# ryienh/gnn-ops-benchmark

Measured on AMD Instinct MI355X. Metric: scatter_add effective HBM GB/s (algorithmic bytes / wall time, cold: index partition + bucketed segment reduce per call), higher is better.
Workload: dtype f32; 1 GPU; c2 (BASELINE configs[1]): torch_scatter.scatter_add(src[E,D], index[E], dim=0, dim_size=N), N=10000000 E=50000000 D=128 fp32, layout R

## Files before the change

gnn-ops-benchmark_amd/csrc/bucket.hip:

```cpp
#include "common.h"
#include "hub.h"
#include "sort_engine.h"

namespace {

constexpr int BSHIFT = 8, BROWS = 1 << BSHIFT;
constexpr int THREADS = 256, WAVES = THREADS / 64;
constexpr int ROUNDS = 16, CAP = THREADS * ROUNDS;
constexpr int U = 8;
constexpr bool NT = true;

inline size_t align_up(size_t v, size_t a) { return (v + a - 1) / a * a; }
inline int key_bits(int64_t N) {
    int bits = 1;
    while (bits < 32 && ((int64_t)1 << bits) < N) ++bits;
    return bits;
}

__global__ void bucket_bounds_kernel(const uint32_t* __restrict__ keys, int64_t E, int64_t NB, int32_t* __restrict__ bptr) {
    const int64_t b = (int64_t)blockIdx.x * blockDim.x + threadIdx.x;
    if (b > NB) return;
    int64_t lo = 0, hi = E;
    while (lo < hi) {
        const int64_t mid = (lo + hi) >> 1;
// ... 337 lines not shown
    if (hub_ws && E > hub::T_HUB) {
        const hub::Layout hl = hub::layout(E, K, want_arg);
        if (hub_ws_bytes >= hl.total) {
            hw = hub::make_ws(hub_ws, hl, E, want_arg);
            if (gnnops_memset_async(hw.counters, 0, 8, stream) != hipSuccess) return gnnops_check_launch("hub memset");
            hub_on = 1;
        }
    }
    hipLaunchKernelGGL((bucket_reduce_kernel<T, R>), dim3(grid), dim3(THREADS), 0, stream, (const T*)src, keys, vals, bptr,
                       (T*)out, arg_out, E, K, N, NB, gshift, kchunks, init_from_out, is_mean, hw, hub_on, spare_keys,
                       spare_vals);
    if (hub_on)
        hub::launch_pass<T, R, true>((const T*)src, nullptr, keys, vals, (T*)out, arg_out, hw, E, K, gshift, kchunks,
                                     init_from_out, is_mean, stream);
    return gnnops_check_launch("scatter_rows_oneshot");
}

template <typename T>
int dispatch_bucket(int reduce, const void* src, const uint32_t* keys, const uint32_t* vals, const int32_t* bptr, void* out,
                    int64_t* arg_out, int64_t E, int64_t K, int64_t N, int64_t NB, int init_from_out, hipStream_t stream,
                    void* hw = nullptr, size_t hb = 0, uint32_t* sk = nullptr, uint32_t* sv = nullptr) {
    switch (reduce) {
        case GNNOPS_SUM: return launch_bucket<T, GNNOPS_SUM>(src, keys, vals, bptr, out, nullptr, E, K, N, NB, init_from_out, 0, stream, hw, hb, sk, sv);
        case GNNOPS_MEAN: return launch_bucket<T, GNNOPS_SUM>(src, keys, vals, bptr, out, nullptr, E, K, N, NB, init_from_out, 1, stream, hw, hb, sk, sv);
        case GNNOPS_MUL: return launch_bucket<T, GNNOPS_MUL>(src, keys, vals, bptr, out, nullptr, E, K, N, NB, init_from_out, 0, stream, hw, hb, sk, sv);
        case GNNOPS_MIN: return launch_bucket<T, GNNOPS_MIN>(src, keys, vals, bptr, out, arg_out, E, K, N, NB, init_from_out, 0, stream, hw, hb, sk, sv);
        case GNNOPS_MAX: return launch_bucket<T, GNNOPS_MAX>(src, keys, vals, bptr, out, arg_out, E, K, N, NB, init_from_out, 0, stream, hw, hb, sk, sv);
    }
    gnnops_set_error("scatter_rows_oneshot: unknown reduce %d", reduce);
    return GNNOPS_EINVAL;
}

struct Layout {
    size_t keys_a, keys_b, vals_a, vals_b, tile_hist, digit_total, bptr, total;
};
inline Layout layout(int64_t E, int64_t N) {
    Layout l{};
    const size_t tiles = (size_t)gnnops_cdiv(E > 0 ? E : 1, sortengine::TILE);
    size_t o = 0;
    l.keys_a = o; o += align_up((size_t)E * 4, 256);
    l.keys_b = o; o += align_up((size_t)E * 4, 256);
    l.vals_a = o; o += align_up((size_t)E * 4, 256);
    l.vals_b = o; o += align_up((size_t)E * 4, 256);
    l.tile_hist = o; o += align_up(256 * tiles * 4, 256);
    l.digit_total = o; o += 256 * 4;
    l.bptr = o; o += align_up(((size_t)gnnops_cdiv(N, BROWS) + 1) * 4, 256);
    l.total = o;
    return l;
}

inline int64_t sentinel_key(int64_t N) { return gnnops_cdiv(N, BROWS) * BROWS; }
inline int partition_passes(int64_t N) { return (key_bits(sentinel_key(N) + 1) - BSHIFT + 7) / 8; }

__global__ void window_keys_kernel(const int64_t* __restrict__ index, uint32_t* __restrict__ keys, int64_t E, int64_t lo,
                                   int64_t N, uint32_t sentinel) {
    for (int64_t e = (int64_t)blockIdx.x * blockDim.x + threadIdx.x; e < E; e += (int64_t)gridDim.x * blockDim.x) {
        const uint64_t d = (uint64_t)(index[e] - lo);
        keys[e] = d < (uint64_t)N ? (uint32_t)d : sentinel;
    }
}

inline bool oneshot_shape_ok(int64_t E, int64_t N) {
    return N > BROWS && E > 0 && E < ((int64_t)1 << 31) && N < ((int64_t)1 << 31);
}

}

extern "C" size_t gnnops_bucket_workspace_bytes(int64_t E, int64_t N) {
    if (E < 0 || N < 0) return 0;
    return layout(E, N).total;
}

namespace {
int partition_impl(const int64_t* index, int64_t E, int64_t lo, int64_t N, bool window, void* workspace,
                   size_t workspace_bytes, hipStream_t stream, const char* what) {
    GNNOPS_REQUIRE(E >= 0 && N >= 0, GNNOPS_EINVAL, "%s: negative size", what);
    GNNOPS_REQUIRE(oneshot_shape_ok(E, N), GNNOPS_EUNSUPPORTED, "%s: shape outside the bucketed form (E=%lld N=%lld)", what,
                   (long long)E, (long long)N);
    GNNOPS_REQUIRE(index, GNNOPS_EINVAL, "%s: null pointer", what);
    const Layout l = layout(E, N);
    GNNOPS_REQUIRE(workspace && workspace_bytes >= l.total, GNNOPS_EWORKSPACE, "%s: workspace %zu < %zu", what,
                   workspace_bytes, l.total);
    char* w = (char*)workspace;
    uint32_t* kbuf[2] = {(uint32_t*)(w + l.keys_a), (uint32_t*)(w + l.keys_b)};
    uint32_t* vbuf[2] = {(uint32_t*)(w + l.vals_a), (uint32_t*)(w + l.vals_b)};
    uint32_t* tile_hist = (uint32_t*)(w + l.tile_hist);
    uint32_t* digit_total = (uint32_t*)(w + l.digit_total);
    int32_t* bptr = (int32_t*)(w + l.bptr);
    const int tiles = (int)gnnops_cdiv(E, sortengine::TILE);
    const int passes = partition_passes(N);
    if (window) {
        const int grid = gnnops_grid_cap(gnnops_cdiv(E, 256), 256 * 16);
        hipLaunchKernelGGL(window_keys_kernel, dim3(grid), dim3(256), 0, stream, index, kbuf[1], E, lo, N,
                           (uint32_t)sentinel_key(N));
    }
    const uint32_t* kin = nullptr;
    const uint32_t* vin = nullptr;
    for (int p = 0; p < passes; ++p) {
        uint32_t* kout = kbuf[p & 1];
        uint32_t* vout = vbuf[p & 1];
        int rc;
        if (p == 0)
            rc = window ? sortengine::pass_first_u32(kbuf[1], kout, vout, E, BSHIFT, tile_hist, digit_total, tiles, stream)
                        : sortengine::pass_first_i64(index, kout, vout, E, BSHIFT, tile_hist, digit_total, tiles, stream);
        else
            rc = sortengine::pass_u32(kin, vin, kout, vout, E, BSHIFT + 8 * p, tile_hist, digit_total, tiles, stream);
        if (rc != GNNOPS_OK) return rc;
        kin = kout; vin = vout;
    }
    const int64_t NB = gnnops_cdiv(N, BROWS);
    hipLaunchKernelGGL(bucket_bounds_kernel, dim3((unsigned)gnnops_cdiv(NB + 1, 256)), dim3(256), 0, stream, kin, E, NB, bptr);
    return gnnops_check_launch(what);
}
}

extern "C" int gnnops_bucket_partition(const int64_t* index, int64_t E, int64_t N, void* workspace, size_t workspace_bytes,
                                       gnnops_stream_t s) {
    return partition_impl(index, E, 0, N, false, workspace, workspace_bytes, (hipStream_t)s, "bucket_partition");
}

extern "C" int gnnops_bucket_partition_window(const int64_t* index, int64_t E, int64_t lo, int64_t N, void* workspace,
                                              size_t workspace_bytes, gnnops_stream_t s) {
    return partition_impl(index, E, lo, N, true, workspace, workspace_bytes, (hipStream_t)s, "bucket_partition_window");
}

extern "C" int gnnops_bucket_layout(int64_t E, int64_t N, size_t* keys_offset, size_t* vals_offset, size_t* bptr_offset) {
    GNNOPS_REQUIRE(E >= 0 && N >= 0 && keys_offset && vals_offset && bptr_offset, GNNOPS_EINVAL, "bucket_layout: bad argument");
    const Layout l = layout(E, N);
    const int last = (partition_passes(N) - 1) & 1;
    *keys_offset = last ? l.keys_b : l.keys_a;
    *vals_offset = last ? l.vals_b : l.vals_a;
    *bptr_offset = l.bptr;
    return GNNOPS_OK;
}

extern "C" int gnnops_bucket_reduce(const void* src, const void* workspace, void* out, int64_t* arg_out, int64_t E, int64_t K,
                                    int64_t N, int dtype, int reduce, int init_from_out, gnnops_stream_t s) {
    return gnnops_bucket_reduce_hubs(src, workspace, out, arg_out, E, K, N, dtype, reduce, init_from_out, nullptr, 0, s);
}

extern "C" int gnnops_bucket_reduce_hubs(const void* src, const void* workspace, void* out, int64_t* arg_out, int64_t E,
                                         int64_t K, int64_t N, int dtype, int reduce, int init_from_out, void* hub_workspace,
                                         size_t hub_workspace_bytes, gnnops_stream_t s) {
    hipStream_t stream = (hipStream_t)s;
    GNNOPS_REQUIRE(E >= 0 && K >= 0 && N >= 0, GNNOPS_EINVAL, "bucket_reduce: negative size");
    GNNOPS_REQUIRE(!(reduce == GNNOPS_MEAN && init_from_out), GNNOPS_EINVAL, "bucket_reduce: mean cannot start from out");
    GNNOPS_REQUIRE(dtype == GNNOPS_F32 || dtype == GNNOPS_F16 || dtype == GNNOPS_BF16, GNNOPS_EINVAL,
                   "bucket_reduce: unknown dtype %d", dtype);
    const int vec = dtype == GNNOPS_F32 ? 4 : 8;
    const bool rows_ok = K > 0 && K % vec == 0 && (uintptr_t)src % 16 == 0 && (uintptr_t)out % 16 == 0 &&
                         (arg_out == nullptr || (uintptr_t)arg_out % 16 == 0);
    GNNOPS_REQUIRE(rows_ok && oneshot_shape_ok(E, N), GNNOPS_EUNSUPPORTED,
                   "bucket_reduce: shape outside the bucketed form (E=%lld K=%lld N=%lld)", (long long)E, (long long)K,
                   (long long)N);
    GNNOPS_REQUIRE(src && workspace && out, GNNOPS_EINVAL, "bucket_reduce: null pointer");
    const Layout l = layout(E, N);
// ... 42 lines not shown
    hub::Ws hw{};
    int hub_on = 0;
    if (hub_workspace && E > hub::T_HUB) {
        const hub::Layout hl = hub::layout(E, 0, false);
        if (hub_workspace_bytes >= hl.total) {
            hw = hub::make_ws(hub_workspace, hl, E, false);
            if (gnnops_memset_async(hw.counters, 0, 8, stream) != hipSuccess) return gnnops_check_launch("hub memset");
            hub_on = 1;
        }
    }
    uint32_t* sk = (uint32_t*)(const_cast<char*>(w) + (last ? l.keys_a : l.keys_b));
    uint32_t* sv = (uint32_t*)(const_cast<char*>(w) + (last ? l.vals_a : l.vals_b));
    hipLaunchKernelGGL((bucket_push_kernel<8>), dim3(grid), dim3(THREADS), 0, stream, (const char*)input, keys, vals, bptr,
                       (char*)out, N, NB, rowbytes, gshift, chunks, hw, hub_on, sk, sv);
    if (hub_on)
        hub::launch_push_pass(true, (const char*)input, nullptr, keys, vals, (char*)out, hw, rowbytes, gshift, chunks, stream);
    return gnnops_check_launch("bucket_select");
}

extern "C" int gnnops_scatter_rows_oneshot(const void* src, const int64_t* index, void* out, int64_t* arg_out, int64_t E,
                                           int64_t K, int64_t N, int dtype, int reduce, int init_from_out,
                                           void* workspace, size_t workspace_bytes, gnnops_stream_t s) {
    GNNOPS_REQUIRE(E >= 0 && K >= 0 && N >= 0, GNNOPS_EINVAL, "scatter_rows_oneshot: negative size");
    const int vec = dtype == GNNOPS_F32 ? 4 : 8;
    const bool rows_ok = K > 0 && K % vec == 0 && (uintptr_t)src % 16 == 0 && (uintptr_t)out % 16 == 0 &&
                         (arg_out == nullptr || (uintptr_t)arg_out % 16 == 0);
    GNNOPS_REQUIRE(rows_ok && oneshot_shape_ok(E, N), GNNOPS_EUNSUPPORTED,
                   "scatter_rows_oneshot: shape outside the one-shot form (E=%lld K=%lld N=%lld)", (long long)E,
                   (long long)K, (long long)N);
    const int rc = gnnops_bucket_partition(index, E, N, workspace, workspace_bytes, s);
    if (rc != GNNOPS_OK) return rc;
    return gnnops_bucket_reduce(src, workspace, out, arg_out, E, K, N, dtype, reduce, init_from_out, s);
}
```

gnn-ops-benchmark_amd/csrc/sort_engine.h:

```cpp
#pragma once
#include "common.h"

namespace sortengine {

constexpr int THREADS = 512;
constexpr int WAVES = THREADS / 64;
constexpr int ROUNDS = 16;
constexpr int TILE = WAVES * ROUNDS * 64;
constexpr int RADIX = 256;

template <typename T>
struct DstValSrc {
    const int64_t* idx;
    const T* val;
    int64_t n_dst;
    uint32_t sentinel;
};

int pass_first_i64(const int64_t* index, uint32_t* keys_out, uint32_t* vals_out, int64_t n, int shift,
                   uint32_t* tile_hist, uint32_t* digit_total, int num_tiles, hipStream_t stream);
int pass_u32(const uint32_t* keys_in, const uint32_t* vals_in, uint32_t* keys_out, uint32_t* vals_out, int64_t n,
             int shift, uint32_t* tile_hist, uint32_t* digit_total, int num_tiles, hipStream_t stream);
int pass_first_u32(const uint32_t* keys_in, uint32_t* keys_out, uint32_t* vals_out, int64_t n, int shift,
                   uint32_t* tile_hist, uint32_t* digit_total, int num_tiles, hipStream_t stream);
int pass_first_f32(const float* keys_in, uint32_t* keys_out, uint32_t* vals_out, int64_t n, int shift,
                   uint32_t* tile_hist, uint32_t* digit_total, int num_tiles, hipStream_t stream);
int pass_first_u64(const uint64_t* keys_in, uint64_t* keys_out, uint32_t* vals_out, int64_t n, int shift,
                   uint32_t* tile_hist, uint32_t* digit_total, int num_tiles, hipStream_t stream);
int pass_u64(const uint64_t* keys_in, const uint32_t* vals_in, uint64_t* keys_out, uint32_t* vals_out, int64_t n,
             int shift, uint32_t* tile_hist, uint32_t* digit_total, int num_tiles, hipStream_t stream);
int pass_first_dstval_f32(const DstValSrc<float>* desc, uint64_t* keys_out, uint32_t* vals_out, int64_t n, int shift,
                          uint32_t* tile_hist, uint32_t* digit_total, int num_tiles, hipStream_t stream);
int pass_first_dstval_f16(const DstValSrc<__half>* desc, uint64_t* keys_out, uint32_t* vals_out, int64_t n, int shift,
                          uint32_t* tile_hist, uint32_t* digit_total, int num_tiles, hipStream_t stream);
int pass_first_dstval_bf16(const DstValSrc<__hip_bfloat16>* desc, uint64_t* keys_out, uint32_t* vals_out, int64_t n, int shift,
                           uint32_t* tile_hist, uint32_t* digit_total, int num_tiles, hipStream_t stream);


}
```

gnn-ops-benchmark_amd/csrc/sort_engine.hip:

```cpp
#include "sort_engine_impl.h"

namespace sortengine {

int pass_first_i64(const int64_t* index, uint32_t* keys_out, uint32_t* vals_out, int64_t n, int shift,
                   uint32_t* tile_hist, uint32_t* digit_total, int num_tiles, hipStream_t stream) {
    return run_pass<KeyI64Low32, true, true>(index, nullptr, keys_out, vals_out, n, shift, tile_hist, digit_total,
                                             num_tiles, stream);
}

int pass_u32(const uint32_t* keys_in, const uint32_t* vals_in, uint32_t* keys_out, uint32_t* vals_out, int64_t n,
             int shift, uint32_t* tile_hist, uint32_t* digit_total, int num_tiles, hipStream_t stream) {
    return run_pass<KeyU32, false, true>(keys_in, vals_in, keys_out, vals_out, n, shift, tile_hist, digit_total,
                                         num_tiles, stream);
}

int pass_first_u32(const uint32_t* keys_in, uint32_t* keys_out, uint32_t* vals_out, int64_t n, int shift,
                   uint32_t* tile_hist, uint32_t* digit_total, int num_tiles, hipStream_t stream) {
    return run_pass<KeyU32, true, true>(keys_in, nullptr, keys_out, vals_out, n, shift, tile_hist, digit_total, num_tiles,
                                        stream);
}

int pass_first_f32(const float* keys_in, uint32_t* keys_out, uint32_t* vals_out, int64_t n, int shift,
                   uint32_t* tile_hist, uint32_t* digit_total, int num_tiles, hipStream_t stream) {
    return run_pass<KeyF32, true, true>(keys_in, nullptr, keys_out, vals_out, n, shift, tile_hist, digit_total,
                                        num_tiles, stream);
}

int pass_first_u64(const uint64_t* keys_in, uint64_t* keys_out, uint32_t* vals_out, int64_t n, int shift,
                   uint32_t* tile_hist, uint32_t* digit_total, int num_tiles, hipStream_t stream) {
    return run_pass<KeyU64, true, true>(keys_in, nullptr, keys_out, vals_out, n, shift, tile_hist, digit_total,
                                        num_tiles, stream);
}

int pass_u64(const uint64_t* keys_in, const uint32_t* vals_in, uint64_t* keys_out, uint32_t* vals_out, int64_t n,
             int shift, uint32_t* tile_hist, uint32_t* digit_total, int num_tiles, hipStream_t stream) {
    return run_pass<KeyU64, false, true>(keys_in, vals_in, keys_out, vals_out, n, shift, tile_hist, digit_total,
                                         num_tiles, stream);
}

int pass_first_dstval_f32(const DstValSrc<float>* desc, uint64_t* keys_out, uint32_t* vals_out, int64_t n, int shift,
                          uint32_t* tile_hist, uint32_t* digit_total, int num_tiles, hipStream_t stream) {
    return run_pass<KeyDstVal<float>, true, true>(desc, nullptr, keys_out, vals_out, n, shift, tile_hist, digit_total, num_tiles, stream);
}

int pass_first_dstval_f16(const DstValSrc<__half>* desc, uint64_t* keys_out, uint32_t* vals_out, int64_t n, int shift,
                          uint32_t* tile_hist, uint32_t* digit_total, int num_tiles, hipStream_t stream) {
    return run_pass<KeyDstVal<__half>, true, true>(desc, nullptr, keys_out, vals_out, n, shift, tile_hist, digit_total, num_tiles, stream);
}

int pass_first_dstval_bf16(const DstValSrc<__hip_bfloat16>* desc, uint64_t* keys_out, uint32_t* vals_out, int64_t n, int shift,
// ... 7 lines not shown
```

gnn-ops-benchmark_amd/csrc/sort_engine_impl.h:

```cpp
#pragma once
#include "common.h"
#include "sort_engine.h"

namespace sortengine {

constexpr int HIST_THREADS = 256;
constexpr int HIST_WAVES = HIST_THREADS / 64;

struct KeyI64Low32 {
    template <typename P> __device__ static inline P open(P p) { return p; }
    using In = int64_t;
    using Carry = uint32_t;
    __device__ static inline Carry load(const In* p, int64_t i) {
        int64_t v = p[i];
        asm("" : "+v"(v));
        return (uint32_t)v;
    }
    __device__ static inline uint32_t digit(Carry k, int shift) { return (k >> shift) & 255u; }
};
struct KeyU32 {
    template <typename P> __device__ static inline P open(P p) { return p; }
    using In = uint32_t;
    using Carry = uint32_t;
    __device__ static inline Carry load(const In* p, int64_t i) { return p[i]; }
// ... 23 lines not shown
        s.n_dst = (uint64_t)p->n_dst;
        s.sentinel = p->sentinel;
        return s;
    }
    __device__ static inline Carry load(const Src& s, int64_t i) {
        const uint64_t d = (uint64_t)s.idx[i];
        float v;
        if constexpr (sizeof(T) == 4) {
            v = *reinterpret_cast<const __attribute__((address_space(1))) float*>(s.val + i);
        } else {
            const uint16_t bits = *reinterpret_cast<const __attribute__((address_space(1))) uint16_t*>(s.val + i);
            T raw;
            __builtin_memcpy(&raw, &bits, 2);
            v = Elem<T>::load(&raw);
        }
        const uint32_t hi = d < s.n_dst ? (uint32_t)d : s.sentinel;
        return ((uint64_t)hi << 32) | (uint64_t)__float_as_uint(v);
    }
    __device__ static inline uint32_t digit(Carry k, int shift) { return (uint32_t)(k >> shift) & 255u; }
};
struct KeyF32 {
    template <typename P> __device__ static inline P open(P p) { return p; }
    using In = float;
    using Carry = uint32_t;
    __device__ static inline Carry load(const In* p, int64_t i) {
        uint32_t u = __float_as_uint(p[i]);
        if (u == 0x80000000u) u = 0u;
        if ((u & 0x7fffffffu) > 0x7f800000u) return 0xffffffffu;
        return (u & 0x80000000u) ? ~u : (u | 0x80000000u);
    }
    __device__ static inline uint32_t digit(Carry k, int shift) { return (k >> shift) & 255u; }
};

template <typename KA>
__global__ __launch_bounds__(HIST_THREADS) void hist_kernel(const typename KA::In* __restrict__ keys_arg, int64_t n,
                                                            int shift, uint32_t* __restrict__ tile_hist,
                                                            int num_tiles) {
    __shared__ uint32_t h[HIST_WAVES][RADIX];
    const int tid = threadIdx.x, wave = tid >> 6;
    for (int i = tid; i < HIST_WAVES * RADIX; i += HIST_THREADS) (&h[0][0])[i] = 0;
    __syncthreads();
    const int tile = (int)xcd_contiguous(blockIdx.x, gridDim.x);
    const int64_t base = (int64_t)tile * TILE;
    const int lim = (int)((n - base < TILE) ? (n - base) : TILE);
    constexpr int GROUPS = TILE / (HIST_THREADS * 4);
    const auto keys = KA::open(keys_arg);
    if (lim == TILE) {
        typename KA::Carry k[GROUPS][4];
#pragma unroll
        for (int g = 0; g < GROUPS; ++g)
#pragma unroll
            for (int j = 0; j < 4; ++j) k[g][j] = KA::load(keys, base + (int64_t)(g * HIST_THREADS + tid) * 4 + j);
#pragma unroll
        for (int g = 0; g < GROUPS; ++g)
#pragma unroll
            for (int j = 0; j < 4; ++j) atomicAdd(&h[wave][KA::digit(k[g][j], shift)], 1u);
    } else {
        for (int i = tid; i < lim; i += HIST_THREADS) atomicAdd(&h[wave][KA::digit(KA::load(keys, base + i), shift)], 1u);
    }
    __syncthreads();
    uint32_t t = 0;
#pragma unroll
    for (int w = 0; w < HIST_WAVES; ++w) t += h[w][tid];
    tile_hist[(size_t)tid * num_tiles + tile] = t;
}

__global__ __launch_bounds__(HIST_THREADS) void scan_kernel(uint32_t* __restrict__ tile_hist, int num_tiles,
                                                            uint32_t* __restrict__ digit_total) {
    __shared__ uint32_t s_tmp[HIST_WAVES];
    uint32_t* row = tile_hist + (size_t)blockIdx.x * num_tiles;
    uint32_t carry = 0;
    constexpr int IPT = 8;
    for (int base = 0; base < num_tiles; base += HIST_THREADS * IPT) {
        uint32_t v[IPT];
        uint32_t sum = 0;
        const int i0 = base + threadIdx.x * IPT;
#pragma unroll
        for (int j = 0; j < IPT; ++j) {
            v[j] = (i0 + j < num_tiles) ? row[i0 + j] : 0u;
            sum += v[j];
        }
        uint32_t tot;
        uint32_t off = carry + block_excl_scan_u32<HIST_WAVES>(sum, s_tmp, &tot);
#pragma unroll
        for (int j = 0; j < IPT; ++j) {
            if (i0 + j < num_tiles) row[i0 + j] = off;
            off += v[j];
        }
        carry += tot;
    }
    if (threadIdx.x == 0) digit_total[blockIdx.x] = carry;
}

template <typename KA, bool IMPLICIT_VALS, bool WRITE_KEYS>
__global__ __launch_bounds__(THREADS, (sizeof(typename KA::Carry) == 4 ? 4 : 2)) void scatter_kernel(const typename KA::In* __restrict__ keys_arg,
                                                          const uint32_t* __restrict__ vals_in,
                                                          typename KA::Carry* __restrict__ keys_out,
                                                          uint32_t* __restrict__ vals_out, int64_t n, int shift,
                                                          const uint32_t* __restrict__ tile_hist_scanned,
                                                          const uint32_t* __restrict__ digit_total, int num_tiles) {
    using Carry = typename KA::Carry;
    constexpr bool PACKED = sizeof(Carry) == 4;
    __shared__ __attribute__((aligned(16))) unsigned char s_image[TILE * (sizeof(Carry) + 4)];
    __shared__ uint32_t s_whist[WAVES][RADIX];
    __shared__ uint32_t s_glob[RADIX];
    __shared__ uint32_t s_tmp[WAVES];
    uint64_t* s_pairs = reinterpret_cast<uint64_t*>(s_image);
    Carry* s_keys = reinterpret_cast<Carry*>(s_image);
    uint32_t* s_vals = reinterpret_cast<uint32_t*>(s_image + TILE * sizeof(Carry));

    const int tid = threadIdx.x, wave = tid >> 6, lane = tid & 63;
    for (int i = tid; i < WAVES * RADIX; i += THREADS) (&s_whist[0][0])[i] = 0;
    __syncthreads();

    const int tile = (int)xcd_contiguous(blockIdx.x, gridDim.x);
    const int64_t base = (int64_t)tile * TILE;
    const int64_t wave_base = base + (int64_t)wave * ROUNDS * 64;
    const uint64_t lanes_below = (lane == 0) ? 0ull : (~0ull >> (64 - lane));
    uint32_t* whist = &s_whist[wave][0];

    Carry key[ROUNDS];
    uint32_t val[ROUNDS];
    const auto keys_in = KA::open(keys_arg);
    if (base + TILE <= n) {
#pragma unroll
        for (int r = 0; r < ROUNDS; ++r) {
            const int64_t i = wave_base + r * 64 + lane;
            key[r] = KA::load(keys_in, i);
            if (!IMPLICIT_VALS) val[r] = vals_in[i];
        }
    } else {
#pragma unroll
        for (int r = 0; r < ROUNDS; ++r) {
            const int64_t i = wave_base + r * 64 + lane;
// ... 61 lines not shown
        if (i < n) {
            const uint32_t d = KA::digit(key[r], shift);
            const uint32_t pos = whist[d] + rank[r];
            const uint32_t v = IMPLICIT_VALS ? (uint32_t)i : val[r];
            if constexpr (PACKED) {
                s_pairs[pos] = ((uint64_t)v << 32) | (uint64_t)(uint32_t)key[r];
            } else {
                s_keys[pos] = key[r];
                s_vals[pos] = v;
            }
        }
    }
    __syncthreads();

    const int lim = (int)((n - base < TILE) ? (n - base) : TILE);
#pragma unroll 4
    for (int i = tid; i < lim; i += THREADS) {
        Carry k;
        uint32_t v;
        if constexpr (PACKED) {
            const uint64_t p = s_pairs[i];
            k = (Carry)(uint32_t)p;
            v = (uint32_t)(p >> 32);
        } else {
            k = s_keys[i];
            v = s_vals[i];
        }
        const uint32_t g = s_glob[KA::digit(k, shift)] + (uint32_t)i;
        if (WRITE_KEYS) keys_out[g] = k;
        vals_out[g] = v;
    }
}

template <typename KA, bool IMPLICIT_VALS, bool WRITE_KEYS>
inline int run_pass(const typename KA::In* keys_in, const uint32_t* vals_in, typename KA::Carry* keys_out,
                    uint32_t* vals_out, int64_t n, int shift, uint32_t* tile_hist, uint32_t* digit_total,
                    int num_tiles, hipStream_t stream) {
    hipLaunchKernelGGL((hist_kernel<KA>), dim3(num_tiles), dim3(HIST_THREADS), 0, stream, keys_in, n, shift,
                       tile_hist, num_tiles);
    hipLaunchKernelGGL(scan_kernel, dim3(RADIX), dim3(HIST_THREADS), 0, stream, tile_hist, num_tiles, digit_total);
    hipLaunchKernelGGL((scatter_kernel<KA, IMPLICIT_VALS, WRITE_KEYS>), dim3(num_tiles), dim3(THREADS), 0, stream,
                       keys_in, vals_in, keys_out, vals_out, n, shift, tile_hist, digit_total, num_tiles);
    return gnnops_check_launch("radix pass");
}

}
```

gnn-ops-benchmark_amd/gnnops/_lib.py:

```python
import ctypes
import os

_HERE = os.path.dirname(os.path.abspath(__file__))
LIB_PATH = os.environ.get("GNNOPS_LIB_PATH") or os.path.join(os.path.dirname(_HERE), "csrc", "libgnnops.so")

ABI_VERSION = 2
F32, F16, BF16 = 0, 1, 2
SUM, MEAN, MIN, MAX, MUL = 0, 1, 2, 3, 4
OK, EINVAL, EWORKSPACE, ELAUNCH, EUNSUPPORTED = 0, 1, 2, 3, 4
ROUTE_NONE, ROUTE_ROWS, ROUTE_K1, ROUTE_LDS, ROUTE_LONGROWS, ROUTE_ELEMS = -1, 0, 1, 2, 3, 4
REDUCE_CODE = {"sum": SUM, "add": SUM, "mean": MEAN, "min": MIN, "max": MAX, "mul": MUL}

_i64, _vp, _ci, _sz = ctypes.c_int64, ctypes.c_void_p, ctypes.c_int, ctypes.c_size_t
SIGNATURES = {
    "gnnops_version": (_ci, []),
    "gnnops_last_error": (ctypes.c_char_p, []),
    "gnnops_diag_stream_mix": (_ci, [_vp, _vp, _i64, _ci, _vp]),
    "gnnops_index_max": (_ci, [_vp, _i64, _vp, _vp]),
    "gnnops_plan_workspace_bytes": (_sz, [_i64, _i64]),
    "gnnops_plan_build": (_ci, [_vp, _i64, _i64, _vp, _vp, _vp, _sz, _vp]),
    "gnnops_plan_small_fits": (_ci, [_i64, _i64]),
    "gnnops_plan_build_small": (_ci, [_vp, _vp, _i64, _i64, _vp, _vp, _vp, _vp]),
    "gnnops_segment_reduce": (_ci, [_vp, _vp, _vp, _vp, _vp, _i64, _i64, _i64, _i64, _ci, _ci, _ci, _vp]),
    "gnnops_bucket_workspace_bytes": (_sz, [_i64, _i64]),
    "gnnops_bucket_partition": (_ci, [_vp, _i64, _i64, _vp, _sz, _vp]),
    "gnnops_bucket_partition_window": (_ci, [_vp, _i64, _i64, _i64, _vp, _sz, _vp]),
    "gnnops_bucket_layout": (_ci, [_i64, _i64, _vp, _vp, _vp]),
    "gnnops_bucket_reduce": (_ci, [_vp, _vp, _vp, _vp, _i64, _i64, _i64, _ci, _ci, _ci, _vp]),
    "gnnops_bucket_reduce_hubs": (_ci, [_vp, _vp, _vp, _vp, _i64, _i64, _i64, _ci, _ci, _ci, _vp, _sz, _vp]),
    "gnnops_hub_workspace_bytes": (_sz, [_i64, _i64, _ci]),
    "gnnops_segment_reduce_hubs": (_ci, [_vp, _vp, _vp, _vp, _vp, _i64, _i64, _i64, _i64, _ci, _ci, _ci, _vp, _sz, _vp]),
    "gnnops_bucket_select_hubs": (_ci, [_vp, _vp, _vp, _i64, _i64, _i64, _ci, _vp, _sz, _vp]),
    "gnnops_index_select_planned_hubs": (_ci, [_vp, _vp, _vp, _vp, _i64, _i64, _i64, _i64, _ci, _vp, _sz, _vp]),
    "gnnops_bucket_select": (_ci, [_vp, _vp, _vp, _i64, _i64, _i64, _ci, _vp]),
    "gnnops_scatter_rows_oneshot": (_ci, [_vp, _vp, _vp, _vp, _i64, _i64, _i64, _ci, _ci, _ci, _vp, _sz, _vp]),
    "gnnops_scatter_elementwise_workspace_bytes": (_sz, [_i64, _i64, _i64, _ci, _ci]),
    "gnnops_scatter_elementwise": (_ci, [_vp, _vp, _vp, _vp, _i64, _i64, _i64, _i64, _ci, _ci, _ci, _vp, _sz, _vp]),
    "gnnops_scatter_elementwise_ix": (_ci, [_vp, _vp, _ci, _vp, _vp, _i64, _i64, _i64, _i64, _ci, _ci, _ci, _vp, _sz, _vp]),
    "gnnops_scatter1d_workspace_bytes": (_sz, [_i64, _i64]),
    "gnnops_scatter1d_minmax": (_ci, [_vp, _vp, _vp, _vp, _i64, _i64, _ci, _ci, _vp, _sz, _vp]),
    "gnnops_scatter1d_sum": (_ci, [_vp, _vp, _vp, _i64, _i64, _ci, _ci, _vp, _sz, _vp]),
    "gnnops_scatter_elementwise_ixa": (_ci, [_vp, _vp, _ci, _vp, _vp, _ci, _i64, _i64, _i64, _i64, _ci, _ci, _ci, _vp, _sz, _vp]),
    "gnnops_transpose2d_cvt": (_ci, [_vp, _vp, _i64, _i64, _ci, _vp]),
    "gnnops_transpose2d_cvt_max": (_ci, [_vp, _vp, _i64, _i64, _vp, _vp]),
    "gnnops_narrow_index": (_ci, [_vp, _vp, _i64, _ci, _i64, _vp]),
    "gnnops_index_select": (_ci, [_vp, _vp, _vp, _i64, _i64, _i64, _i64, _ci, _vp]),
    "gnnops_index_select_planned": (_ci, [_vp, _vp, _vp, _vp, _i64, _i64, _i64, _i64, _ci, _vp]),
    "gnnops_gather": (_ci, [_vp, _vp, _vp, _i64, _i64, _i64, _i64, _ci, _vp]),
    "gnnops_fused_select_sum_workspace_bytes": (_sz, []),
    "gnnops_fused_index_select_sum": (_ci, [_vp, _vp, _vp, _i64, _i64, _i64, _i64, _ci, _vp, _sz, _vp]),
    "gnnops_index_select_route": (_ci, [_i64, _i64, _i64, _i64, _ci, _sz, _sz, ctypes.POINTER(_ci)]),
    "gnnops_gather_route": (_ci, [_i64, _i64, _i64, _i64, _ci, ctypes.POINTER(_ci)]),
    "gnnops_fused_select_sum_route": (_ci, [_i64, _i64, _i64, _i64, _ci, _sz, ctypes.POINTER(_ci)]),
    "gnnops_spmm": (_ci, [_vp, _vp, _vp, _vp, _vp, _vp, _i64, _i64, _i64, _i64, _ci, _vp]),
    "gnnops_spmm_hubs": (_ci, [_vp, _vp, _vp, _vp, _vp, _vp, _i64, _i64, _i64, _i64, _ci, _vp, _sz, _vp]),
    "gnnops_spmm_tiled": (_ci, [_vp, _vp, _vp, _vp, _vp, _i64, _i64, _i64, _ci, _vp, _vp, _vp, _ci, _ci, _vp]),
    "gnnops_permute": (_ci, [_vp, _vp, _vp, _i64, _ci, _vp]),
    "gnnops_sort_workspace_bytes": (_sz, [_i64, _i64, _i64, _ci]),
    "gnnops_sort": (_ci, [_vp, _vp, _vp, _i64, _i64, _i64, _ci, _ci, _vp, _sz, _vp]),
    "gnnops_sort_rows_max_len": (_i64, []),
# ... 83 lines not shown
```

include/gnnops.h:

```cpp
#ifndef GNNOPS_H
#define GNNOPS_H

#include <stddef.h>
#include <stdint.h>

#ifdef __cplusplus
extern "C" {
#endif

#define GNNOPS_ABI_VERSION 2

enum gnnops_status {
    GNNOPS_OK = 0,
    GNNOPS_EINVAL = 1,
    GNNOPS_EWORKSPACE = 2,
    GNNOPS_ELAUNCH = 3,
    GNNOPS_EUNSUPPORTED = 4
};

enum gnnops_dtype { GNNOPS_F32 = 0, GNNOPS_F16 = 1, GNNOPS_BF16 = 2 };

enum gnnops_reduce { GNNOPS_SUM = 0, GNNOPS_MEAN = 1, GNNOPS_MIN = 2, GNNOPS_MAX = 3, GNNOPS_MUL = 4 };

typedef void* gnnops_stream_t;
// ... 2 lines not shown
const char* gnnops_last_error(void);

int gnnops_diag_stream_mix(const void* src, void* dst, int64_t pieces, int reads, gnnops_stream_t stream);

int gnnops_index_max(const int64_t* index, int64_t E, int64_t* d_max, gnnops_stream_t stream);

size_t gnnops_plan_workspace_bytes(int64_t E, int64_t N);
int gnnops_plan_build(const int64_t* index, int64_t E, int64_t N,
                      int32_t* rowptr, int32_t* perm,
                      void* workspace, size_t workspace_bytes, gnnops_stream_t stream);
int gnnops_plan_small_fits(int64_t E, int64_t N);
int gnnops_plan_build_small(const int64_t* index, const int64_t* companion, int64_t E, int64_t N, int32_t* rowptr,
                            int32_t* perm, int64_t* col, gnnops_stream_t stream);

int gnnops_segment_reduce(const void* src, const int32_t* rowptr, const int32_t* perm,
                          void* out, int64_t* arg_out,
                          int64_t B, int64_t E, int64_t K, int64_t N,
                          int dtype, int reduce, int init_from_out, gnnops_stream_t stream);
size_t gnnops_hub_workspace_bytes(int64_t E, int64_t K, int reduce);
int gnnops_segment_reduce_hubs(const void* src, const int32_t* rowptr, const int32_t* perm,
                               void* out, int64_t* arg_out,
                               int64_t B, int64_t E, int64_t K, int64_t N,
                               int dtype, int reduce, int init_from_out,
                               void* hub_workspace, size_t hub_workspace_bytes, gnnops_stream_t stream);

int gnnops_scatter_rows_oneshot(const void* src, const int64_t* index, void* out, int64_t* arg_out,
                                int64_t E, int64_t K, int64_t N, int dtype, int reduce, int init_from_out,
                                void* workspace, size_t workspace_bytes, gnnops_stream_t stream);
size_t gnnops_bucket_workspace_bytes(int64_t E, int64_t N);
int gnnops_bucket_partition(const int64_t* index, int64_t E, int64_t N, void* workspace, size_t workspace_bytes,
                            gnnops_stream_t stream);
int gnnops_bucket_partition_window(const int64_t* index, int64_t E, int64_t lo, int64_t N, void* workspace,
                                   size_t workspace_bytes, gnnops_stream_t stream);
int gnnops_bucket_layout(int64_t E, int64_t N, size_t* keys_offset, size_t* vals_offset, size_t* bptr_offset);
int gnnops_bucket_reduce(const void* src, const void* workspace, void* out, int64_t* arg_out,
                         int64_t E, int64_t K, int64_t N, int dtype, int reduce, int init_from_out,
                         gnnops_stream_t stream);
int gnnops_bucket_reduce_hubs(const void* src, const void* workspace, void* out, int64_t* arg_out,
                              int64_t E, int64_t K, int64_t N, int dtype, int reduce, int init_from_out,
                              void* hub_workspace, size_t hub_workspace_bytes, gnnops_stream_t stream);
int gnnops_bucket_select(const void* input, const void* workspace, void* out, int64_t N, int64_t K, int64_t E,
                         int elem_bytes, gnnops_stream_t stream);
int gnnops_bucket_select_hubs(const void* input, const void* workspace, void* out, int64_t N, int64_t K, int64_t E,
                              int elem_bytes, void* hub_workspace, size_t hub_workspace_bytes, gnnops_stream_t stream);
int gnnops_index_select_planned_hubs(const void* input, const int32_t* rowptr, const int32_t* perm, void* out,
                                     int64_t B, int64_t N, int64_t K, int64_t E, int elem_bytes,
                                     void* hub_workspace, size_t hub_workspace_bytes, gnnops_stream_t stream);

size_t gnnops_scatter_elementwise_workspace_bytes(int64_t B, int64_t N, int64_t K, int dtype, int reduce);
int gnnops_scatter_elementwise(const void* src, const int64_t* index, void* out, int64_t* arg_out,
                               int64_t B, int64_t E, int64_t K, int64_t N,
                               int dtype, int reduce, int init_from_out,
                               void* workspace, size_t workspace_bytes, gnnops_stream_t stream);
int gnnops_scatter_elementwise_ix(const void* src, const void* index, int index_bytes, void* out, int64_t* arg_out,
                                  int64_t B, int64_t E, int64_t K, int64_t N, int dtype, int reduce, int init_from_out,
                                  void* workspace, size_t workspace_bytes, gnnops_stream_t stream);
int gnnops_scatter_elementwise_ixa(const void* src, const void* index, int index_bytes, void* out, void* arg_out, int arg_bytes,
                                   int64_t B, int64_t E, int64_t K, int64_t N, int dtype, int reduce, int init_from_out,
                                   void* workspace, size_t workspace_bytes, gnnops_stream_t stream);
int gnnops_narrow_index(const int64_t* index, void* out, int64_t n, int out_bytes, int64_t bound, gnnops_stream_t stream);

size_t gnnops_scatter1d_workspace_bytes(int64_t E, int64_t N);
int gnnops_scatter1d_minmax(const void* src, const int64_t* index, void* out, int64_t* arg_out, int64_t E, int64_t N,
                            int dtype, int reduce, void* workspace, size_t workspace_bytes, gnnops_stream_t stream);
int gnnops_scatter1d_sum(const void* src, const int64_t* index, void* out, int64_t E, int64_t N, int dtype, int reduce,
                         void* workspace, size_t workspace_bytes, gnnops_stream_t stream);
// ... 169 lines not shown
```

Before: 4806 GB/s.

## Detect already-sorted index during first radix histogram and skip remaining sort work

```diff
diff --git a/gnn-ops-benchmark_amd/csrc/bucket.hip b/gnn-ops-benchmark_amd/csrc/bucket.hip
--- a/gnn-ops-benchmark_amd/csrc/bucket.hip
+++ b/gnn-ops-benchmark_amd/csrc/bucket.hip
@@ -393,7 +393,7 @@
 }
 
 struct Layout {
-    size_t keys_a, keys_b, vals_a, vals_b, tile_hist, digit_total, bptr, total;
+    size_t keys_a, keys_b, vals_a, vals_b, tile_hist, digit_total, bptr, tile_ordered, ordered_flag, total;
 };
 inline Layout layout(int64_t E, int64_t N) {
     Layout l{};
@@ -406,6 +406,8 @@
     l.tile_hist = o; o += align_up(256 * tiles * 4, 256);
     l.digit_total = o; o += 256 * 4;
     l.bptr = o; o += align_up(((size_t)gnnops_cdiv(N, BROWS) + 1) * 4, 256);
+    l.tile_ordered = o; o += align_up(tiles * 4, 256);
+    l.ordered_flag = o; o += 256;
     l.total = o;
     return l;
 }
@@ -420,6 +422,9 @@
         keys[e] = d < (uint64_t)N ? (uint32_t)d : sentinel;
     }
 }
+
+int launch_identity_fill(bool window, const int64_t* index, const uint32_t* wkeys, uint32_t* keys, uint32_t* vals, int64_t E,
+                         const uint32_t* ordered, hipStream_t stream);
 
 inline bool oneshot_shape_ok(int64_t E, int64_t N) {
     return N > BROWS && E > 0 && E < ((int64_t)1 << 31) && N < ((int64_t)1 << 31);
@@ -448,6 +453,8 @@
     uint32_t* tile_hist = (uint32_t*)(w + l.tile_hist);
     uint32_t* digit_total = (uint32_t*)(w + l.digit_total);
     int32_t* bptr = (int32_t*)(w + l.bptr);
+    uint32_t* tile_ordered = (uint32_t*)(w + l.tile_ordered);
+    uint32_t* ordered = (uint32_t*)(w + l.ordered_flag);
     const int tiles = (int)gnnops_cdiv(E, sortengine::TILE);
     const int passes = partition_passes(N);
     if (window) {
@@ -462,13 +469,14 @@
         uint32_t* vout = vbuf[p & 1];
         int rc;
         if (p == 0)
-            rc = window ? sortengine::pass_first_u32(kbuf[1], kout, vout, E, BSHIFT, tile_hist, digit_total, tiles, stream)
-                        : sortengine::pass_first_i64(index, kout, vout, E, BSHIFT, tile_hist, digit_total, tiles, stream);
+            rc = window ? sortengine::pass_first_u32(kbuf[1], kout, vout, E, BSHIFT, tile_hist, digit_total, tiles, stream, tile_ordered, ordered)
+                        : sortengine::pass_first_i64(index, kout, vout, E, BSHIFT, tile_hist, digit_total, tiles, stream, tile_ordered, ordered);
         else
-            rc = sortengine::pass_u32(kin, vin, kout, vout, E, BSHIFT + 8 * p, tile_hist, digit_total, tiles, stream);
+            rc = sortengine::pass_u32(kin, vin, kout, vout, E, BSHIFT + 8 * p, tile_hist, digit_total, tiles, stream, ordered);
         if (rc != GNNOPS_OK) return rc;
         kin = kout; vin = vout;
     }
+    launch_identity_fill(window, index, kbuf[1], const_cast<uint32_t*>(kin), const_cast<uint32_t*>(vin), E, ordered, stream);
     const int64_t NB = gnnops_cdiv(N, BROWS);
     hipLaunchKernelGGL(bucket_bounds_kernel, dim3((unsigned)gnnops_cdiv(NB + 1, 256)), dim3(256), 0, stream, kin, E, NB, bptr);
     return gnnops_check_launch(what);
@@ -483,6 +491,17 @@
 extern "C" int gnnops_bucket_partition_window(const int64_t* index, int64_t E, int64_t lo, int64_t N, void* workspace,
                                               size_t workspace_bytes, gnnops_stream_t s) {
     return partition_impl(index, E, lo, N, true, workspace, workspace_bytes, (hipStream_t)s, "bucket_partition_window");
+}
+
+extern "C" int gnnops_bucket_partition_was_identity(const void* workspace, int64_t E, int64_t N, int* out, gnnops_stream_t s) {
+    GNNOPS_REQUIRE(workspace && out && oneshot_shape_ok(E, N), GNNOPS_EINVAL, "bucket_partition_was_identity: bad argument");
+    const Layout l = layout(E, N);
+    uint32_t flag = 0;
+    GNNOPS_REQUIRE(hipStreamSynchronize((hipStream_t)s) == hipSuccess &&
+                       hipMemcpy(&flag, (const char*)workspace + l.ordered_flag, 4, hipMemcpyDeviceToHost) == hipSuccess,
+                   GNNOPS_ELAUNCH, "bucket_partition_was_identity: reading the flag failed");
+    *out = flag != 0;
+    return GNNOPS_OK;
 }
 
 extern "C" int gnnops_bucket_layout(int64_t E, int64_t N, size_t* keys_offset, size_t* vals_offset, size_t* bptr_offset) {
@@ -591,3 +610,44 @@
     if (rc != GNNOPS_OK) return rc;
     return gnnops_bucket_reduce(src, workspace, out, arg_out, E, K, N, dtype, reduce, init_from_out, s);
 }
+
+namespace {
+template <bool WINDOW>
+__global__ __launch_bounds__(256) void identity_fill_kernel(const int64_t* __restrict__ index, const uint32_t* wkeys,
+                                                            uint32_t* keys, uint32_t* __restrict__ vals, int64_t E,
+                                                            const uint32_t* __restrict__ ordered) {
+    if (*ordered == 0) return;
+    const int64_t quads = E >> 2;
+    const bool copy_keys = wkeys != keys;
+    for (int64_t q = (int64_t)blockIdx.x * blockDim.x + threadIdx.x; q < quads; q += (int64_t)gridDim.x * blockDim.x) {
+        const int64_t e = q * 4;
+        if (copy_keys) {
+            u32x4 k;
+            if constexpr (WINDOW) {
+                k = *reinterpret_cast<const u32x4*>(wkeys + e);
+            } else {
+                k.x = (uint32_t)index[e]; k.y = (uint32_t)index[e + 1]; k.z = (uint32_t)index[e + 2]; k.w = (uint32_t)index[e + 3];
+            }
+            *reinterpret_cast<u32x4*>(keys + e) = k;
+        }
+        u32x4 v;
+        v.x = (uint32_t)e; v.y = (uint32_t)e + 1; v.z = (uint32_t)e + 2; v.w = (uint32_t)e + 3;
+        *reinterpret_cast<u32x4*>(vals + e) = v;
+    }
+    const int64_t e = quads * 4 + threadIdx.x;
+    if (blockIdx.x == 0 && threadIdx.x < 4 && e < E) {
+        if (copy_keys) keys[e] = WINDOW ? wkeys[e] : (uint32_t)index[e];
+        vals[e] = (uint32_t)e;
+    }
+}
+
+int launch_identity_fill(bool window, const int64_t* index, const uint32_t* wkeys, uint32_t* keys, uint32_t* vals, int64_t E,
+                         const uint32_t* ordered, hipStream_t stream) {
+    const dim3 grid(gnnops_grid_cap(gnnops_cdiv(E, 256 * 4), 256 * 16));
+    if (window)
+        hipLaunchKernelGGL(identity_fill_kernel<true>, grid, dim3(256), 0, stream, index, wkeys, keys, vals, E, ordered);
+    else
+        hipLaunchKernelGGL(identity_fill_kernel<false>, grid, dim3(256), 0, stream, index, (const uint32_t*)nullptr, keys, vals, E, ordered);
+    return GNNOPS_OK;
+}
+}
diff --git a/gnn-ops-benchmark_amd/csrc/sort_engine.h b/gnn-ops-benchmark_amd/csrc/sort_engine.h
--- a/gnn-ops-benchmark_amd/csrc/sort_engine.h
+++ b/gnn-ops-benchmark_amd/csrc/sort_engine.h
@@ -18,11 +18,14 @@
 };
 
 int pass_first_i64(const int64_t* index, uint32_t* keys_out, uint32_t* vals_out, int64_t n, int shift,
-                   uint32_t* tile_hist, uint32_t* digit_total, int num_tiles, hipStream_t stream);
+                   uint32_t* tile_hist, uint32_t* digit_total, int num_tiles, hipStream_t stream,
+                   uint32_t* tile_ordered = nullptr, uint32_t* ordered_flag = nullptr);
 int pass_u32(const uint32_t* keys_in, const uint32_t* vals_in, uint32_t* keys_out, uint32_t* vals_out, int64_t n,
-             int shift, uint32_t* tile_hist, uint32_t* digit_total, int num_tiles, hipStream_t stream);
+             int shift, uint32_t* tile_hist, uint32_t* digit_total, int num_tiles, hipStream_t stream,
+             const uint32_t* skip = nullptr);
 int pass_first_u32(const uint32_t* keys_in, uint32_t* keys_out, uint32_t* vals_out, int64_t n, int shift,
-                   uint32_t* tile_hist, uint32_t* digit_total, int num_tiles, hipStream_t stream);
+                   uint32_t* tile_hist, uint32_t* digit_total, int num_tiles, hipStream_t stream,
+                   uint32_t* tile_ordered = nullptr, uint32_t* ordered_flag = nullptr);
 int pass_first_f32(const float* keys_in, uint32_t* keys_out, uint32_t* vals_out, int64_t n, int shift,
                    uint32_t* tile_hist, uint32_t* digit_total, int num_tiles, hipStream_t stream);
 int pass_first_u64(const uint64_t* keys_in, uint64_t* keys_out, uint32_t* vals_out, int64_t n, int shift,
diff --git a/gnn-ops-benchmark_amd/csrc/sort_engine.hip b/gnn-ops-benchmark_amd/csrc/sort_engine.hip
--- a/gnn-ops-benchmark_amd/csrc/sort_engine.hip
+++ b/gnn-ops-benchmark_amd/csrc/sort_engine.hip
@@ -3,19 +3,27 @@
 namespace sortengine {
 
 int pass_first_i64(const int64_t* index, uint32_t* keys_out, uint32_t* vals_out, int64_t n, int shift,
-                   uint32_t* tile_hist, uint32_t* digit_total, int num_tiles, hipStream_t stream) {
+                   uint32_t* tile_hist, uint32_t* digit_total, int num_tiles, hipStream_t stream, uint32_t* tile_ordered,
+                   uint32_t* ordered_flag) {
+    if (tile_ordered && ordered_flag)
+        return run_pass<KeyI64Low32, true, true, true>(index, nullptr, keys_out, vals_out, n, shift, tile_hist, digit_total,
+                                                       num_tiles, stream, tile_ordered, ordered_flag);
     return run_pass<KeyI64Low32, true, true>(index, nullptr, keys_out, vals_out, n, shift, tile_hist, digit_total,
                                              num_tiles, stream);
 }
 
 int pass_u32(const uint32_t* keys_in, const uint32_t* vals_in, uint32_t* keys_out, uint32_t* vals_out, int64_t n,
-             int shift, uint32_t* tile_hist, uint32_t* digit_total, int num_tiles, hipStream_t stream) {
+             int shift, uint32_t* tile_hist, uint32_t* digit_total, int num_tiles, hipStream_t stream, const uint32_t* skip) {
     return run_pass<KeyU32, false, true>(keys_in, vals_in, keys_out, vals_out, n, shift, tile_hist, digit_total,
-                                         num_tiles, stream);
+                                         num_tiles, stream, nullptr, nullptr, skip);
 }
 
 int pass_first_u32(const uint32_t* keys_in, uint32_t* keys_out, uint32_t* vals_out, int64_t n, int shift,
-                   uint32_t* tile_hist, uint32_t* digit_total, int num_tiles, hipStream_t stream) {
+                   uint32_t* tile_hist, uint32_t* digit_total, int num_tiles, hipStream_t stream, uint32_t* tile_ordered,
+                   uint32_t* ordered_flag) {
+    if (tile_ordered && ordered_flag)
+        return run_pass<KeyU32, true, true, true>(keys_in, nullptr, keys_out, vals_out, n, shift, tile_hist, digit_total,
+                                                  num_tiles, stream, tile_ordered, ordered_flag);
     return run_pass<KeyU32, true, true>(keys_in, nullptr, keys_out, vals_out, n, shift, tile_hist, digit_total, num_tiles,
                                         stream);
 }
diff --git a/gnn-ops-benchmark_amd/csrc/sort_engine_impl.h b/gnn-ops-benchmark_amd/csrc/sort_engine_impl.h
--- a/gnn-ops-benchmark_amd/csrc/sort_engine_impl.h
+++ b/gnn-ops-benchmark_amd/csrc/sort_engine_impl.h
@@ -79,42 +79,111 @@
     __device__ static inline uint32_t digit(Carry k, int shift) { return (k >> shift) & 255u; }
 };
 
-template <typename KA>
+template <typename KA, bool DETECT = false>
 __global__ __launch_bounds__(HIST_THREADS) void hist_kernel(const typename KA::In* __restrict__ keys_arg, int64_t n,
                                                             int shift, uint32_t* __restrict__ tile_hist,
-                                                            int num_tiles) {
+                                                            int num_tiles, uint32_t* __restrict__ tile_ordered,
+                                                            const uint32_t* __restrict__ skip) {
+    constexpr int GROUPS = TILE / (HIST_THREADS * 4);
+    constexpr int SEAMS = GROUPS * HIST_WAVES;
+    static_assert(!DETECT || (sizeof(typename KA::Carry) == 4 && SEAMS <= 64), "order test: u32 carries, seams fit one wave");
     __shared__ uint32_t h[HIST_WAVES][RADIX];
+    __shared__ uint32_t s_first[DETECT ? SEAMS : 1], s_last[DETECT ? SEAMS : 1], s_wbad[HIST_WAVES];
+    if (skip && *skip) return;
     const int tid = threadIdx.x, wave = tid >> 6;
     for (int i = tid; i < HIST_WAVES * RADIX; i += HIST_THREADS) (&h[0][0])[i] = 0;
     __syncthreads();
     const int tile = (int)xcd_contiguous(blockIdx.x, gridDim.x);
     const int64_t base = (int64_t)tile * TILE;
     const int lim = (int)((n - base < TILE) ? (n - base) : TILE);
-    constexpr int GROUPS = TILE / (HIST_THREADS * 4);
     const auto keys = KA::open(keys_arg);
+    [[maybe_unused]] bool bad = false;
+    [[maybe_unused]] uint32_t seam = ~0u;
     if (lim == TILE) {
         typename KA::Carry k[GROUPS][4];
-#pragma unroll
-        for (int g = 0; g < GROUPS; ++g)
+        [[maybe_unused]] uint32_t first[GROUPS], last[GROUPS];
+        constexpr int AHEAD = DETECT ? GROUPS - 2 : GROUPS;
+#pragma unroll
+        for (int g = 0; g < AHEAD; ++g)
 #pragma unroll
             for (int j = 0; j < 4; ++j) k[g][j] = KA::load(keys, base + (int64_t)(g * HIST_THREADS + tid) * 4 + j);
-#pragma unroll
-        for (int g = 0; g < GROUPS; ++g)
+        if constexpr (DETECT) {
+            const bool more = base + TILE < n;
+            const uint32_t s = (uint32_t)keys_arg[more ? base + TILE : base] >> shift;
+            seam = more ? s : ~0u;
+        }
+#pragma unroll
+        for (int g = 0; g < GROUPS; ++g) {
 #pragma unroll
             for (int j = 0; j < 4; ++j) atomicAdd(&h[wave][KA::digit(k[g][j], shift)], 1u);
+            if constexpr (DETECT) {
+                const uint32_t a0 = k[g][0] >> shift, a1 = k[g][1] >> shift, a2 = k[g][2] >> shift, a3 = k[g][3] >> shift;
+                const uint32_t prev = (uint32_t)__builtin_amdgcn_update_dpp((int)a0, (int)a3, 0x138, 0xf, 0xf, false);
+                bad |= (a0 > a1) | (a1 > a2) | (a2 > a3) | (prev > a0);
+                first[g] = (uint32_t)__builtin_amdgcn_readfirstlane((int)a0);
+                last[g] = (uint32_t)__builtin_amdgcn_readlane((int)a3, 63);
+                if (g + AHEAD < GROUPS) {
+                    __builtin_amdgcn_sched_barrier(0);
+#pragma unroll
+                    for (int j = 0; j < 4; ++j)
+                        k[g + AHEAD][j] = KA::load(keys, base + (int64_t)((g + AHEAD) * HIST_THREADS + tid) * 4 + j);
+                    __builtin_amdgcn_sched_barrier(0);
+                }
+            }
+        }
+        if constexpr (DETECT) {
+            const int g_mine = tid & 63;
+            if (g_mine < GROUPS) {
+                uint32_t fv = first[0], lv = last[0];
+#pragma unroll
+                for (int g = 1; g < GROUPS; ++g) {
+                    fv = g_mine == g ? first[g] : fv;
+                    lv = g_mine == g ? last[g] : lv;
+                }
+                s_first[g_mine * HIST_WAVES + wave] = fv;
+                s_last[g_mine * HIST_WAVES + wave] = lv;
+            }
+        }
+    } else if constexpr (DETECT) {
+        for (int i0 = 0; i0 < lim; i0 += HIST_THREADS) {
+            const int i = i0 + tid;
+            const bool valid = i < lim, has_next = i + 1 < lim;
+            const typename KA::Carry kk = valid ? KA::load(keys, base + i) : (typename KA::Carry)0;
+            if (valid) atomicAdd(&h[wave][KA::digit(kk, shift)], 1u);
+            const uint32_t a = kk >> shift;
+            uint32_t nxt = __shfl_down(a, 1);
+            if ((tid & 63) == 63 && has_next) nxt = (uint32_t)(KA::load(keys, base + i + 1) >> shift);
+            bad |= has_next && a > nxt;
+        }
     } else {
         for (int i = tid; i < lim; i += HIST_THREADS) atomicAdd(&h[wave][KA::digit(KA::load(keys, base + i), shift)], 1u);
     }
+    if constexpr (DETECT) {
+        const bool wbad = __ballot(bad) != 0;
+        if ((tid & 63) == 0) s_wbad[wave] = wbad ? 1u : 0u;
+    }
     __syncthreads();
     uint32_t t = 0;
 #pragma unroll
     for (int w = 0; w < HIST_WAVES; ++w) t += h[w][tid];
     tile_hist[(size_t)tid * num_tiles + tile] = t;
+    if constexpr (DETECT) {
+        if (wave == 0) {
+            bool sb = tid < HIST_WAVES && s_wbad[tid] != 0;
+            if (lim == TILE && tid < SEAMS) sb |= s_last[tid] > (tid + 1 < SEAMS ? s_first[tid + 1] : seam);
+            const bool any = __ballot(sb) != 0;
+            if (tid == 0) tile_ordered[tile] = any ? 0u : 1u;
+        }
+    }
 }
 
 __global__ __launch_bounds__(HIST_THREADS) void scan_kernel(uint32_t* __restrict__ tile_hist, int num_tiles,
-                                                            uint32_t* __restrict__ digit_total) {
+                                                            uint32_t* __restrict__ digit_total,
+                                                            const uint32_t* __restrict__ tile_ordered,
+                                                            uint32_t* __restrict__ ordered_flag,
+                                                            const uint32_t* __restrict__ skip) {
     __shared__ uint32_t s_tmp[HIST_WAVES];
+    if (skip && *skip) return;
     uint32_t* row = tile_hist + (size_t)blockIdx.x * num_tiles;
     uint32_t carry = 0;
     constexpr int IPT = 8;
@@ -137,6 +206,12 @@
         carry += tot;
     }
     if (threadIdx.x == 0) digit_total[blockIdx.x] = carry;
+    if (tile_ordered && blockIdx.x == 0) {
+        int bad = 0;
+        for (int i = threadIdx.x; i < num_tiles; i += HIST_THREADS) bad |= tile_ordered[i] == 0u;
+        bad = __syncthreads_or(bad);
+        if (threadIdx.x == 0) *ordered_flag = bad ? 0u : 1u;
+    }
 }
 
 template <typename KA, bool IMPLICIT_VALS, bool WRITE_KEYS>
@@ -145,8 +220,10 @@
                                                           typename KA::Carry* __restrict__ keys_out,
                                                           uint32_t* __restrict__ vals_out, int64_t n, int shift,
                                                           const uint32_t* __restrict__ tile_hist_scanned,
-                                                          const uint32_t* __restrict__ digit_total, int num_tiles) {
+                                                          const uint32_t* __restrict__ digit_total, int num_tiles,
+                                                          const uint32_t* __restrict__ skip) {
     using Carry = typename KA::Carry;
+    if (skip && *skip) return;
     constexpr bool PACKED = sizeof(Carry) == 4;
     __shared__ __attribute__((aligned(16))) unsigned char s_image[TILE * (sizeof(Carry) + 4)];
     __shared__ uint32_t s_whist[WAVES][RADIX];
@@ -274,15 +351,18 @@
     }
 }
 
-template <typename KA, bool IMPLICIT_VALS, bool WRITE_KEYS>
+template <typename KA, bool IMPLICIT_VALS, bool WRITE_KEYS, bool DETECT = false>
 inline int run_pass(const typename KA::In* keys_in, const uint32_t* vals_in, typename KA::Carry* keys_out,
                     uint32_t* vals_out, int64_t n, int shift, uint32_t* tile_hist, uint32_t* digit_total,
-                    int num_tiles, hipStream_t stream) {
-    hipLaunchKernelGGL((hist_kernel<KA>), dim3(num_tiles), dim3(HIST_THREADS), 0, stream, keys_in, n, shift,
-                       tile_hist, num_tiles);
-    hipLaunchKernelGGL(scan_kernel, dim3(RADIX), dim3(HIST_THREADS), 0, stream, tile_hist, num_tiles, digit_total);
+                    int num_tiles, hipStream_t stream, uint32_t* tile_ordered = nullptr, uint32_t* ordered_flag = nullptr,
+                    const uint32_t* skip = nullptr) {
+    hipLaunchKernelGGL((hist_kernel<KA, DETECT>), dim3(num_tiles), dim3(HIST_THREADS), 0, stream, keys_in, n, shift,
+                       tile_hist, num_tiles, tile_ordered, skip);
+    hipLaunchKernelGGL(scan_kernel, dim3(RADIX), dim3(HIST_THREADS), 0, stream, tile_hist, num_tiles, digit_total,
+                       (const uint32_t*)tile_ordered, ordered_flag, skip);
     hipLaunchKernelGGL((scatter_kernel<KA, IMPLICIT_VALS, WRITE_KEYS>), dim3(num_tiles), dim3(THREADS), 0, stream,
-                       keys_in, vals_in, keys_out, vals_out, n, shift, tile_hist, digit_total, num_tiles);
+                       keys_in, vals_in, keys_out, vals_out, n, shift, tile_hist, digit_total, num_tiles,
+                       DETECT ? (const uint32_t*)ordered_flag : skip);
     return gnnops_check_launch("radix pass");
 }
 
diff --git a/gnn-ops-benchmark_amd/gnnops/_lib.py b/gnn-ops-benchmark_amd/gnnops/_lib.py
--- a/gnn-ops-benchmark_amd/gnnops/_lib.py
+++ b/gnn-ops-benchmark_amd/gnnops/_lib.py
@@ -26,6 +26,7 @@
     "gnnops_bucket_partition": (_ci, [_vp, _i64, _i64, _vp, _sz, _vp]),
     "gnnops_bucket_partition_window": (_ci, [_vp, _i64, _i64, _i64, _vp, _sz, _vp]),
     "gnnops_bucket_layout": (_ci, [_i64, _i64, _vp, _vp, _vp]),
+    "gnnops_bucket_partition_was_identity": (_ci, [_vp, _i64, _i64, ctypes.POINTER(_ci), _vp]),
     "gnnops_bucket_reduce": (_ci, [_vp, _vp, _vp, _vp, _i64, _i64, _i64, _ci, _ci, _ci, _vp]),
     "gnnops_bucket_reduce_hubs": (_ci, [_vp, _vp, _vp, _vp, _i64, _i64, _i64, _ci, _ci, _ci, _vp, _sz, _vp]),
     "gnnops_hub_workspace_bytes": (_sz, [_i64, _i64, _ci]),
diff --git a/include/gnnops.h b/include/gnnops.h
--- a/include/gnnops.h
+++ b/include/gnnops.h
@@ -58,6 +58,7 @@
                             gnnops_stream_t stream);
 int gnnops_bucket_partition_window(const int64_t* index, int64_t E, int64_t lo, int64_t N, void* workspace,
                                    size_t workspace_bytes, gnnops_stream_t stream);
+int gnnops_bucket_partition_was_identity(const void* workspace, int64_t E, int64_t N, int* out, gnnops_stream_t stream);
 int gnnops_bucket_layout(int64_t E, int64_t N, size_t* keys_offset, size_t* vals_offset, size_t* bptr_offset);
 int gnnops_bucket_reduce(const void* src, const void* workspace, void* out, int64_t* arg_out,
                          int64_t E, int64_t K, int64_t N, int dtype, int reduce, int init_from_out,
```

Result: no change. 4790 GB/s (-0.3%).
